# charlesq34/pointnet2

Hardware: AMD Instinct MI355X
Metric: point-clouds/sec for SA(FPS+ball+group) B=32 N=4096→1024 nsample=32 (higher is better)
Workload: dtype f32

## Files before the change

pointnet2_amd/csrc/fps_batch_body.h:

```cpp
#pragma once
#include "fps_pruned_body.h"

namespace pn2 {

constexpr int kBtCand = PN2_WAVE;
constexpr int kBtMaxW = 8;
#ifndef PN2_BT_UT
#define PN2_BT_UT 512
#endif
constexpr int kBtUT = PN2_BT_UT;
constexpr int kBtT = kBtUT + PN2_WAVE;
constexpr unsigned kBtEnd = 0x100u, kBtFill = 0x200u, kBtCountMask = 0xffu;

struct BtXchg {
    double list[kBtCand];
    unsigned cnt[kBtMaxW];
    unsigned bound[kBtMaxW];
    unsigned bmax;
    unsigned total;
    unsigned count;
    unsigned spare0;
    unsigned single;
    unsigned theta, vlast;
    unsigned spare1;
};
static_assert(sizeof(BtXchg) == 8 * kBtCand + 8 * kBtMaxW + 32, "the size the LDS budget of every geometry was measured with");
static_assert(sizeof(BtXchg) % 16 == 0 && offsetof(BtXchg, bmax) % 16 == 0, "16-byte rows");

__host__ __device__ constexpr size_t fps_batch_xchg_offset(int P, int UT = kBtUT) { return (fps_pruned_lds_bytes(P, UT) + 15) & ~(size_t)15; }
__host__ __device__ constexpr size_t fps_batch_lds_bytes(int P, int UT = kBtUT) { return fps_batch_xchg_offset(P, UT) + 2 * sizeof(BtXchg) + 16 * kBtCand; }

__device__ __forceinline__ float vmax_f32(float a, float b)
{
    float r;
    asm("v_max_f32 %0, %1, %2" : "=v"(r) : "v"(a), "v"(b));
    return r;
}
__device__ __forceinline__ float vmed3_f32(float a, float b, float c)
{
    float r;
    asm("v_med3_f32 %0, %1, %2, %3" : "=v"(r) : "v"(a), "v"(b), "v"(c));
    return r;
}

__device__ __forceinline__ int bt_wave_max_i32_lane63(int v)
{
#define PN2_BT_STEP(ctrl) v = max(v, __builtin_amdgcn_update_dpp(0, v, ctrl, 0xf, 0xf, true))
    PN2_BT_STEP(0xB1);
    PN2_BT_STEP(0x4E);
    PN2_BT_STEP(0x141);
    PN2_BT_STEP(0x140);
    PN2_BT_STEP(0x142);
    PN2_BT_STEP(0x143);
#undef PN2_BT_STEP
    return v;
}

__device__ __forceinline__ double kBtInvalidKey() { return -1.0; }

__device__ __forceinline__ void lds_max_u32(unsigned *p, unsigned v)
{
    asm volatile("ds_max_u32 %0, %1" :: "v"((unsigned)(size_t)p), "v"(v) : "memory");
}

__device__ __forceinline__ void lds_add_u32(unsigned *p, unsigned v)
{
    asm volatile("ds_add_u32 %0, %1" :: "v"((unsigned)(size_t)p), "v"(v) : "memory");
}

inline bool fps_batch_covers(int ranks) { return ranks > 512 && ranks <= 8192; }
#ifdef PN2_BT_LAB_NEVER_AUTO
inline bool fps_batch_pays(int, int) { return false; }
#else
inline bool fps_batch_pays(int ranks, int m) { return fps_batch_covers(ranks) && m >= 256; }
#endif

#ifdef PN2_BT_STATS
__device__ unsigned long long g_bt_stats[16];
#ifndef PN2_BT_STATS_FROM
#define PN2_BT_STATS_FROM 0
#endif
#define PN2_BT_STAT(i, v) do { if (lane == 0 && cloud == 0 && j >= PN2_BT_STATS_FROM) atomicAdd(&g_bt_stats[i], (unsigned long long)(v)); } while (0)
#define PN2_BT_CLOCK() __builtin_readcyclecounter()
#else
#define PN2_BT_STAT(i, v) do { } while (0)
#define PN2_BT_CLOCK() 0ll
#pragma clang diagnostic ignored "-Wunused-variable"
#endif

#ifndef PN2_BT_LIST_HI
#define PN2_BT_LIST_HI 36
#define PN2_BT_LIST_LO 20
#endif
#ifndef PN2_BT_EARLY
#define PN2_BT_EARLY 48
#endif
#ifndef PN2_BT_ASM_LOOP
#define PN2_BT_ASM_LOOP 1
#endif
#ifndef PN2_BT_RFL
#define PN2_BT_RFL 1
#endif
#ifndef PN2_BT_NOCTR
#define PN2_BT_NOCTR 1
#endif
#ifndef PN2_BT_FILL
#define PN2_BT_FILL 1
#endif
#ifndef PN2_BT_READ1
#define PN2_BT_READ1 1
#endif
#ifndef PN2_BT_CADD
#define PN2_BT_CADD 1
#endif
#ifndef PN2_BT_G0
#define PN2_BT_G0 0.10f
#endif
#ifndef PN2_BT_PACKED_FROM
#define PN2_BT_PACKED_FROM 16
#endif
#ifndef PN2_BT_SLOW_MIN
#define PN2_BT_SLOW_MIN 3
#define PN2_BT_QUICK 1
#define PN2_BT_SINGLE0 16
#define PN2_BT_SINGLE1 512
#endif

template <int P, int GS, bool PUBLISH, int UT = kBtUT>
__device__ __forceinline__ void fps_batch_body(int n, int m, int Q, int cloud, const float *__restrict__ xyz,
                                               int *__restrict__ out, float *__restrict__ out_xyz,
                                               unsigned long long *__restrict__ tagged, char *smem, unsigned tag = 1u)
{
    constexpr int W = UT / PN2_WAVE, NS = UT * P;
    constexpr int GW = P / GS;
    constexpr int CAP = kBtCand / W;
    constexpr int BT = UT + PN2_WAVE;
    static_assert((W * GW == 32 && (W == 4 || W == 8)) || (W == 8 && (GW == 2 || GW == 1)),
                  "32 groups on four or eight updater waves; 16 / 8 groups (2048 / 1024 rank slots) on eight");
    float4 *lds_rank = reinterpret_cast<float4 *>(smem + 256);
    BtXchg *xch = reinterpret_cast<BtXchg *>(smem + fps_batch_xchg_offset(P, UT));
    float4 *ring = reinterpret_cast<float4 *>(smem + fps_batch_xchg_offset(P, UT) + 2 * sizeof(BtXchg));

    const float *__restrict__ src = xyz + (size_t)cloud * n * 3;
    int *__restrict__ dst = out + (size_t)cloud * m;
    float *__restrict__ dxyz = out_xyz ? out_xyz + (size_t)cloud * m * 3 : nullptr;
    pn2_gu64 *gtag = PUBLISH ? (pn2_gu64 *)(tagged + (size_t)cloud * m) : nullptr;
    const int t = threadIdx.x;
    const int lane = t & 63;
    const int w = __builtin_amdgcn_readfirstlane(t >> 6);

    int j = 1;
    const int jE = min(PN2_BT_EARLY, m);
    int fill_k = -1;

    if (w == W) {
#ifndef PN2_NO_SETPRIO
        __builtin_amdgcn_s_setprio(3);
#endif
        for (int i = lane; i < (int)(2 * sizeof(BtXchg) / 4); i += PN2_WAVE) reinterpret_cast<unsigned *>(xch)[i] = 0u;
#if PN2_BT_READ1
        xch[0].list[lane] = kBtInvalidKey();
        xch[1].list[lane] = kBtInvalidKey();
#endif
        for (int i = 0; i < kPrPrologueBarriers; ++i) __syncthreads();
        long long e0 = 0;
        for (; j < jE; ++j) {
            if (j == 8) e0 = (long long)__builtin_readcyclecounter();
            __syncthreads();
        }
        const float round_cyc = jE >= 24 ? (float)((long long)__builtin_readcyclecounter() - e0) / (float)(jE - 8) : 1e30f;
        float bt_cyc = 0.f, bt_smp = 0.f;
        int bt_n = 0, bt_paid = 0, run = PN2_BT_SINGLE0, a_prev = 0, single_next = 0;
        long long qb = 0;
        float g = PN2_BT_G0;
        int par = 0;
        if (j < m)
        for (;;) {
            const long long q0 = PN2_BT_CLOCK();
#if PN2_BT_READ1
            xch[par ^ 1].list[lane] = kBtInvalidKey();
#endif
            {
                const long long qn = (long long)__builtin_readcyclecounter();
                if (bt_n > 0) {
                    bt_cyc = 0.75f * bt_cyc + (float)(qn - qb); bt_smp = 0.75f * bt_smp + (float)a_prev;
                    if (bt_n > PN2_BT_QUICK) {
                        if (bt_cyc > bt_smp * round_cyc * (bt_n > PN2_BT_SLOW_MIN ? 1.0f : 1.5f)) {
                            single_next = run;
                            run = min(2 * run, PN2_BT_SINGLE1);
                            bt_n = -1; bt_paid = 0; bt_cyc = 0.f; bt_smp = 0.f;
                        } else if (++bt_paid >= 8) {
                            run = PN2_BT_SINGLE0;
                        }
                    }
                }
                qb = qn;
                ++bt_n;
            }
            __syncthreads();
            const long long q1 = PN2_BT_CLOCK();
            BtXchg &X = xch[par];
            typedef float bt_f4 __attribute__((ext_vector_type(4)));
#if PN2_BT_READ1
            if (lane == 0) *reinterpret_cast<uint4 *>(&xch[par ^ 1].bmax) = make_uint4(0u, 0u, 0u, 0u);
            const uint2 bt2 = *reinterpret_cast<const uint2 *>(&X.bmax);
            const double key = X.list[lane];
            const unsigned lowc = (unsigned)__double2loint(key);
            const bt_f4 cand = *reinterpret_cast<const bt_f4 *>(&lds_rank[lowc]);
            const int boundb = __builtin_amdgcn_readfirstlane((int)bt2.x);
            const int total = __builtin_amdgcn_readfirstlane((int)bt2.y);
            int cval = __double2hiint(key);
#else
            if (lane == 0) __hip_atomic_store(&xch[par ^ 1].count, 0u, __ATOMIC_RELAXED, __HIP_MEMORY_SCOPE_WORKGROUP);
            const uint4 c4 = *reinterpret_cast<const uint4 *>(X.cnt), c5 = *reinterpret_cast<const uint4 *>(X.cnt + 4);
            const uint4 b4 = *reinterpret_cast<const uint4 *>(X.bound), b5 = *reinterpret_cast<const uint4 *>(X.bound + 4);
            const double key = X.list[lane];
            const unsigned cw = X.cnt[lane / CAP];
            const bool valid = (unsigned)(lane & (CAP - 1)) < cw;
            const unsigned lowc = valid ? (unsigned)__double2loint(key) : 0u;
            const bt_f4 cand = *reinterpret_cast<const bt_f4 *>(&lds_rank[lowc]);
            const int boundb = __builtin_amdgcn_readfirstlane((int)max(max(max(b4.x, b4.y), max(b4.z, b4.w)), max(max(b5.x, b5.y), max(b5.z, b5.w))));
            const int total = __builtin_amdgcn_readfirstlane((int)(c4.x + c4.y + c4.z + c4.w + c5.x + c5.y + c5.z + c5.w));
            int cval = valid ? __double2hiint(key) : (int)0xBF800000;
#endif
            const int clo = (int)lowc;
            int a = 0;
            int vlastb = 0;
            bool fill = false;
            const unsigned ring_base = (unsigned)(size_t)ring, count_addr = (unsigned)(size_t)&X.count;
            const long long q2 = PN2_BT_CLOCK();
            int bh;
            unsigned long long eq;
            auto argmax = [&]() __attribute__((always_inline)) {
                bh = __builtin_amdgcn_readlane(bt_wave_max_i32_lane63(cval), 63);
                eq = __ballot(cval == bh);
                if (__popcll(eq) != 1) {
                    PN2_BT_STAT(11, 1);
                    const double kq = cval == bh ? __hiloint2double(cval, clo) : -1.0;
                    const double km = wave_max_f64_lane63(kq);
                    const int ml = __builtin_amdgcn_readlane(__double2loint(km), 63);
                    eq = __ballot(cval == bh && clo == ml);
                    eq &= 0ull - eq;
                }
            };
            argmax();
            const int amax = min(m - j, kBtCand);
            unsigned raddr = ring_base, na = 1u;
            auto pick_counted = [&]() __attribute__((always_inline)) {
                for (;;) {
                    asm volatile("s_mov_b64 exec, %1\n\t"
                                 "ds_write_b128 %2, %3\n\t"
                                 "ds_write_b32 %4, %5\n\t"
                                 "v_mov_b32 %0, 0xbf800000\n\t"
                                 "s_mov_b64 exec, -1"
                                 : "+v"(cval) : "s"(eq), "v"(raddr), "v"(cand), "v"(count_addr), "v"(na) : "memory");
                    const int wl = (int)__builtin_ctzll(eq);
                    raddr += 16u; na += 1u;
                    a = __builtin_amdgcn_readfirstlane(a + 1);
                    vlastb = bh;
                    if (a >= amax) break;
                    const int ms = __builtin_amdgcn_readlane(bt_wave_max_i32_lane63(cval), 63);
                    const float sx = __int_as_float(__builtin_amdgcn_readlane(__float_as_int(cand.x), wl));
                    const float sy = __int_as_float(__builtin_amdgcn_readlane(__float_as_int(cand.y), wl));
                    const float sz = __int_as_float(__builtin_amdgcn_readlane(__float_as_int(cand.z), wl));
                    const float d = sqdist(cand.x, cand.y, cand.z, sx, sy, sz);
                    cval = __float_as_int(vmin_f32(d, __int_as_float(cval)));
                    if (ms < boundb) break;
                    eq = __ballot(cval == ms);
                    bh = ms;
                    if (__popcll(eq) != 1) {
                        PN2_BT_STAT(12, 1);
                        argmax();
                        if (bh < boundb) break;
                    }
                }
            };
#if PN2_BT_ASM_LOOP
#if PN2_BT_RFL
#define PN2_BT_A_WINNER_IN  "v_readfirstlane_b32 %[sx], %[cx]\n\tv_readfirstlane_b32 %[sy], %[cy]\n\tv_readfirstlane_b32 %[sz], %[cz]\n\t"
#define PN2_BT_A_LANE       ""
#define PN2_BT_A_SXY        ""
#define PN2_BT_A_SZ         ""
#else
#define PN2_BT_A_WINNER_IN  ""
#define PN2_BT_A_LANE       "s_ff1_i32_b64 %[wl], %[eq]\n\t"
#define PN2_BT_A_SXY        "v_readlane_b32 %[sx], %[cx], %[wl]\n\tv_readlane_b32 %[sy], %[cy], %[wl]\n\t"
#define PN2_BT_A_SZ         "v_readlane_b32 %[sz], %[cz], %[wl]\n\t"
#endif
#if PN2_BT_NOCTR
#define PN2_BT_A_COUNT      ""
#define PN2_BT_A_FULL       ""
#else
#define PN2_BT_A_COUNT      "s_add_i32 %[a], %[a], 1\n\t"
#define PN2_BT_A_FULL       "s_cmp_ge_i32 %[a], %[amax]\n\ts_cbranch_scc1 2f\n\t"
#endif
#if PN2_BT_CADD
#define PN2_BT_A_PUBCOUNT   "ds_add_u32 %[caddr], %[one]\n\t"
#define PN2_BT_A_NA         ""
#else
#define PN2_BT_A_PUBCOUNT   "ds_write_b32 %[caddr], %[na]\n\t"
#define PN2_BT_A_NA         "v_add_u32 %[na], 1, %[na]\n\t"
#endif
#if PN2_BT_CADD && PN2_BT_FILL
#define PN2_BT_A_HEAD       "0:\n\t"
#define PN2_BT_A_BH         "s_mov_b32 %[bh], %[ms]\n\t"
#define PN2_BT_A_MS         "+s"
#else
#define PN2_BT_A_HEAD       "s_branch 1f\n\t0:\n\ts_mov_b32 %[bh], %[ms]\n\t1:\n\t"
#define PN2_BT_A_BH         ""
#define PN2_BT_A_MS         "=&s"
#endif
#if PN2_BT_FILL
#define PN2_BT_A_ADDS_EARLY ""
#define PN2_BT_A_PAD_DPP    "v_add_u32 %[raddr], 16, %[raddr]\n\t" PN2_BT_A_NA PN2_BT_A_BH
#define PN2_BT_A_PAD        ""
#else
#define PN2_BT_A_ADDS_EARLY "v_add_u32 %[raddr], 16, %[raddr]\n\t" PN2_BT_A_NA
#define PN2_BT_A_PAD_DPP    "s_nop 1\n\t"
#define PN2_BT_A_PAD        "s_nop 0\n\t"
#endif
            const float cx = cand.x, cy = cand.y, cz = cand.z;
#if PN2_BT_NOCTR
            if (amax < kBtCand) pick_counted();
            else
#endif
            for (;;) {
                int reason, t_wl, t_sx, t_sy, t_sz, t_cnt;
                int t_ms = bh;
                int v_t;
                float v_dx, v_dy, v_dz;
                asm volatile(
                    PN2_BT_A_HEAD
                    "s_mov_b64 exec, %[eq]\n\t"
                    "ds_write_b128 %[raddr], %[cand]\n\t"
                    PN2_BT_A_PUBCOUNT
                    "v_mov_b32 %[cval], 0xbf800000\n\t"
                    PN2_BT_A_WINNER_IN
                    "s_mov_b64 exec, -1\n\t"
                    PN2_BT_A_LANE
                    PN2_BT_A_COUNT
                    PN2_BT_A_ADDS_EARLY
                    PN2_BT_A_FULL
                    PN2_BT_A_SXY
                    "v_max_i32_dpp %[t], %[cval], %[cval] quad_perm:[1,0,3,2] row_mask:0xf bank_mask:0xf bound_ctrl:0\n\t"
                    PN2_BT_A_SZ
                    "v_subrev_f32 %[dx], %[sx], %[cx]\n\t"
                    "v_subrev_f32 %[dy], %[sy], %[cy]\n\t"
                    "v_max_i32_dpp %[t], %[t], %[t] quad_perm:[2,3,0,1] row_mask:0xf bank_mask:0xf bound_ctrl:0\n\t"
                    "v_subrev_f32 %[dz], %[sz], %[cz]\n\t"
                    "v_mul_f32 %[dx], %[dx], %[dx]\n\t"
                    "v_max_i32_dpp %[t], %[t], %[t] row_half_mirror row_mask:0xf bank_mask:0xf bound_ctrl:0\n\t"
                    "v_mul_f32 %[dy], %[dy], %[dy]\n\t"
                    "v_mul_f32 %[dz], %[dz], %[dz]\n\t"
                    "v_max_i32_dpp %[t], %[t], %[t] row_mirror row_mask:0xf bank_mask:0xf bound_ctrl:0\n\t"
                    "v_add_f32 %[dx], %[dx], %[dy]\n\t"
                    "v_add_f32 %[dx], %[dx], %[dz]\n\t"
                    "v_max_i32_dpp %[t], %[t], %[t] row_bcast:15 row_mask:0xf bank_mask:0xf bound_ctrl:0\n\t"
                    PN2_BT_A_PAD_DPP
                    "v_max_i32_dpp %[t], %[t], %[t] row_bcast:31 row_mask:0xf bank_mask:0xf bound_ctrl:0\n\t"
                    "v_min_f32 %[cval], %[dx], %[cval]\n\t"
                    PN2_BT_A_PAD
                    "v_readlane_b32 %[ms], %[t], 63\n\t"
                    PN2_BT_A_PAD
                    "s_cmp_lt_i32 %[ms], %[bound]\n\t"
                    "s_cbranch_scc1 3f\n\t"
                    "v_cmp_eq_u32_e64 %[eq], %[ms], %[cval]\n\t"
                    "s_bcnt1_i32_b64 %[cnt], %[eq]\n\t"
                    "s_cmp_eq_u32 %[cnt], 1\n\t"
                    "s_cbranch_scc1 0b\n\t"
                    "s_mov_b32 %[reason], 2\n\t"
                    "s_branch 4f\n\t"
#if !PN2_BT_NOCTR
                    "2:\n\t"
                    "s_mov_b32 %[reason], 0\n\t"
                    "s_branch 4f\n\t"
#endif
                    "3:\n\t"
                    "s_mov_b32 %[reason], 1\n\t"
                    "4:"
                    : [cval] "+v"(cval), [raddr] "+v"(raddr), [na] "+v"(na), [eq] "+s"(eq), [bh] "+s"(bh),
#if !PN2_BT_NOCTR
                      [a] "+s"(a),
#endif
                      [reason] "=&s"(reason), [wl] "=&s"(t_wl), [sx] "=&s"(t_sx), [sy] "=&s"(t_sy), [sz] "=&s"(t_sz), [ms] PN2_BT_A_MS(t_ms), [cnt] "=&s"(t_cnt),
                      [t] "=&v"(v_t), [dx] "=&v"(v_dx), [dy] "=&v"(v_dy), [dz] "=&v"(v_dz)
                    : [cand] "v"(cand), [caddr] "v"(count_addr), [cx] "v"(cx), [cy] "v"(cy), [cz] "v"(cz), [amax] "s"(amax), [bound] "s"(boundb), [one] "v"(1u)
                    : "memory", "scc");
                vlastb = bh;
                if (reason != 2) break;
                PN2_BT_STAT(12, 1);
                argmax();
                if (bh < boundb) break;
            }
#if PN2_BT_NOCTR
#if PN2_BT_CADD
            a = (int)((unsigned)__builtin_amdgcn_readfirstlane((int)raddr) - ring_base) >> 4;
#else
            a = __builtin_amdgcn_readfirstlane((int)na) - 1;
#endif
#endif
#undef PN2_BT_A_WINNER_IN
#undef PN2_BT_A_LANE
#undef PN2_BT_A_SXY
#undef PN2_BT_A_SZ
#undef PN2_BT_A_COUNT
#undef PN2_BT_A_FULL
#undef PN2_BT_A_PUBCOUNT
#undef PN2_BT_A_NA
#undef PN2_BT_A_HEAD
#undef PN2_BT_A_BH
#undef PN2_BT_A_MS
#undef PN2_BT_A_ADDS_EARLY
#undef PN2_BT_A_PAD_DPP
#undef PN2_BT_A_PAD
#else
            pick_counted();
#endif
            if (vlastb == 0) { fill = true; fill_k = __builtin_amdgcn_readlane(__float_as_int(cand.w), (int)__builtin_ctzll(eq)); }
            const long long q3 = PN2_BT_CLOCK();
            if (total > PN2_BT_LIST_HI) g = fmaxf(g * 0.8f, 1.0f / 128.0f);
            else if (total < PN2_BT_LIST_LO) g = fminf(g * 1.25f, 0.5f);
            X.theta = __float_as_uint(__fmul_rn(__int_as_float(vlastb), 1.0f - g));
            X.vlast = (unsigned)vlastb;
            a_prev = a;
            int single = min(single_next, m - (j + a));
            if (single_next) { PN2_BT_STAT(13, single); PN2_BT_STAT(14, 1); }
            single_next = 0;
            single = __builtin_amdgcn_readfirstlane(single);
            X.single = (unsigned)single;
            if (lane == 0)
                __hip_atomic_store(&X.count, (unsigned)a | kBtEnd | (fill ? kBtFill : 0u), __ATOMIC_RELEASE, __HIP_MEMORY_SCOPE_WORKGROUP);
            PN2_BT_STAT(0, 1); PN2_BT_STAT(1, a); PN2_BT_STAT(4, total); PN2_BT_STAT(6, q2 - q1); PN2_BT_STAT(7, q3 - q2); PN2_BT_STAT(8, q1 - q0);
            j = __builtin_amdgcn_readfirstlane(j + a);
            if (fill || j >= m) break;
            for (int i = 0; i < single; ++i) __syncthreads();
            j += single;
            if (j >= m) break;
            par ^= 1;
        }
    } else {
        PrSlots<P> S;
        fps_pruned_prologue<P, GS, UT>(n, Q, src, smem, S);
        pn2_f2 (&xx)[P / 2] = S.xx;
        pn2_f2 (&yy)[P / 2] = S.yy;
        pn2_f2 (&zz)[P / 2] = S.zz;
        float (&md)[P] = S.md;
        unsigned (&low)[P] = S.low;
        float blx, bly, blz, bhx, bhy, bhz;
        {
            const float *gbox = reinterpret_cast<const float *>(smem + 256 + (size_t)16 * NS + (size_t)kPrHistRows * kPrBins * 4);
            const float *o = gbox + (w * GW + (lane & (GW - 1))) * 8;
            blx = o[0]; bly = o[1]; blz = o[2]; bhx = o[4]; bhy = o[5]; bhz = o[6];
        }
        pn2_f2 sxy = {0.f, 0.f}, syy = {0.f, 0.f}, szk = {0.f, 0.f};
        auto update_group = [&](auto gic) __attribute__((always_inline)) {
            constexpr int gi = decltype(gic)::value;
            constexpr int H = GS / 2;
            pn2_f2 dx[H], dy[H], dz[H];
#pragma unroll
            for (int h = 0; h < H; ++h) dx[h] = pk_sub_bcast_lo(xx[gi * H + h], sxy);
#pragma unroll
            for (int h = 0; h < H; ++h) dy[h] = pk_sub_bcast_lo(yy[gi * H + h], syy);
#pragma unroll
            for (int h = 0; h < H; ++h) dz[h] = pk_sub_bcast_lo(zz[gi * H + h], szk);
#pragma unroll
            for (int h = 0; h < H; ++h) dx[h] = pk_mul(dx[h], dx[h]);
#pragma unroll
            for (int h = 0; h < H; ++h) dy[h] = pk_mul(dy[h], dy[h]);
#pragma unroll
            for (int h = 0; h < H; ++h) dz[h] = pk_mul(dz[h], dz[h]);
#pragma unroll
            for (int h = 0; h < H; ++h) dx[h] = pk_add(dx[h], dy[h]);
#pragma unroll
            for (int h = 0; h < H; ++h) dx[h] = pk_add(dx[h], dz[h]);
#pragma unroll
            for (int h = 0; h < H; ++h) {
                const int p0 = gi * GS + 2 * h;
                md[p0] = vmin_f32(dx[h].x, md[p0]);
                md[p0 + 1] = vmin_f32(dx[h].y, md[p0 + 1]);
            }
        };
        auto update_all = [&]() __attribute__((always_inline)) {
            update_group(std::integral_constant<int, 0>());
            if constexpr (GW >= 2) update_group(std::integral_constant<int, 1>());
            if constexpr (GW >= 4) { update_group(std::integral_constant<int, 2>()); update_group(std::integral_constant<int, 3>()); }
            if constexpr (GW == 8) {
                update_group(std::integral_constant<int, 4>()); update_group(std::integral_constant<int, 5>());
                update_group(std::integral_constant<int, 6>()); update_group(std::integral_constant<int, 7>());
            }
        };
        {
            const float4 s = lds_rank[NS - 1];
            sxy.x = s.x; syy.x = s.y; szk.x = s.z;
            update_all();
        }
        if (t == 0) {
            dst[0] = 0;
            if (PUBLISH) __hip_atomic_store(gtag, (unsigned long long)tag << 32, __ATOMIC_RELAXED, __HIP_MEMORY_SCOPE_AGENT);
        }
        unsigned vlastb = __float_as_uint(1e38f);
        unsigned thetab = __float_as_uint(1e38f);
        auto single_rounds = [&](const int jend) __attribute__((always_inline)) {
            double *partial = reinterpret_cast<double *>(smem);
            for (; j < jend; ++j) {
                double kd[P];
#pragma unroll
                for (int p = 0; p < P; ++p) kd[p] = __hiloint2double(__float_as_int(md[p]), (int)low[p]);
#pragma unroll
                for (int st = 1; st < P; st <<= 1)
#pragma unroll
                    for (int i = 0; i + st < P; i += 2 * st)
                        asm("v_max_f64 %0, %1, %2" : "=v"(kd[i]) : "v"(kd[i]), "v"(kd[i + st]));
                const double wd = wave_max_f64_lane63(kd[0]);
                double *slot = partial + (j & 1) * W;
                if (lane == 63) slot[w] = wd;
                __syncthreads();
                double key[W];
#pragma unroll
                for (int i = 0; i < W; ++i) key[i] = slot[i];
#pragma unroll
                for (int st = 1; st < W; st <<= 1)
#pragma unroll
                    for (int i = 0; i + st < W; i += 2 * st)
                        asm("v_max_f64 %0, %1, %2" : "=v"(key[i]) : "v"(key[i]), "v"(key[i + st]));
                vlastb = (unsigned)__double2hiint(key[0]);
                const float4 s = lds_rank[(unsigned)__double2loint(key[0])];
                if (t == 0) {
                    const int k = __float_as_int(s.w);
                    dst[j] = k;
                    if (PUBLISH)
                        __hip_atomic_store(gtag + j, ((unsigned long long)tag << 32) | (unsigned long long)(unsigned)k, __ATOMIC_RELAXED,
                                           __HIP_MEMORY_SCOPE_AGENT);
                }
                if constexpr (P >= PN2_BT_PACKED_FROM) {
                    sxy.x = s.x; syy.x = s.y; szk.x = s.z;
                    update_all();
                } else {
#pragma unroll
                    for (int p = 0; p < P; ++p) {
                        const float d = p & 1 ? sqdist(xx[p / 2].y, yy[p / 2].y, zz[p / 2].y, s.x, s.y, s.z)
                                              : sqdist(xx[p / 2].x, yy[p / 2].x, zz[p / 2].x, s.x, s.y, s.z);
                        md[p] = vmin_f32(d, md[p]);
                    }
                }
            }
            thetab = __float_as_uint(__fmul_rn(__uint_as_float(vlastb), 1.0f - PN2_BT_G0));
        };
        if (jE > 1) single_rounds(jE);
        int par = 0;
        if (j < m)
        for (;;) {
            BtXchg &X = xch[par];
            const long long u0 = PN2_BT_CLOCK();
            double kl;
            float sec;
            {
                double kd[P];
                float hv[P / 2], lv[P / 2];
#pragma unroll
                for (int p = 0; p < P; ++p) kd[p] = __hiloint2double(__float_as_int(md[p]), (int)low[p]);
#pragma unroll
                for (int i = 0; i < P / 2; ++i) { hv[i] = vmax_f32(md[2 * i], md[2 * i + 1]); lv[i] = vmin_f32(md[2 * i], md[2 * i + 1]); }
#pragma unroll
                for (int st = 1; st < P; st <<= 1)
#pragma unroll
                    for (int i = 0; i + st < P; i += 2 * st)
                        asm("v_max_f64 %0, %1, %2" : "=v"(kd[i]) : "v"(kd[i]), "v"(kd[i + st]));
#pragma unroll
                for (int st = 1; st < P / 2; st <<= 1)
#pragma unroll
                    for (int i = 0; i + st < P / 2; i += 2 * st) {
                        const float ll = vmax_f32(lv[i], lv[i + st]);
                        lv[i] = vmed3_f32(hv[i], hv[i + st], ll);
                        hv[i] = vmax_f32(hv[i], hv[i + st]);
                    }
                kl = kd[0];
                sec = lv[0];
            }
            const unsigned vb = (unsigned)__double2hiint(kl);
            unsigned long long mask = __ballot(vb >= thetab);
            int cnt = __popcll(mask);
            unsigned thb = thetab;
            bool exact = false;
            if (cnt > CAP) {
                unsigned lob = thetab, hib = vlastb + 1u;
                for (int it = 0; it < 16; ++it) {
                    const unsigned mid = lob + ((hib - lob) >> 1);
                    if (mid == lob) break;
                    const unsigned long long mk = __ballot(vb >= mid);
                    const int c = __popcll(mk);
                    PN2_BT_STAT(3, 1);
                    if (c > CAP) lob = mid;
                    else if (c == 0) hib = mid;
                    else { mask = mk; cnt = c; thb = mid; break; }
                }
                exact = cnt > CAP;
            } else if (cnt == 0) {
                exact = true;
            }
            if (exact) {
                PN2_BT_STAT(2, 1);
                const double wk = wave_max_f64_lane63(kl);
                const int bh = __builtin_amdgcn_readlane(__double2hiint(wk), 63), bl = __builtin_amdgcn_readlane(__double2loint(wk), 63);
                unsigned long long mk = __ballot(__double2hiint(kl) == bh && __double2loint(kl) == bl);
                mk &= 0ull - mk;
                if (cnt != 0) thb = (unsigned)bh + 1u;
                mask = mk;
                cnt = 1;
            }
            if ((mask >> lane) & 1ull) {
                const int pos = __builtin_amdgcn_mbcnt_hi((unsigned)(mask >> 32), __builtin_amdgcn_mbcnt_lo((unsigned)mask, 0u));
                X.list[w * CAP + pos] = kl;
#if PN2_BT_READ1
                lds_max_u32(&X.bmax, __float_as_uint(sec) + 1u);
#else
                lds_max_u32(&X.bound[w], __float_as_uint(sec) + 1u);
#endif
            }
            if (lane == 0) {
#if PN2_BT_READ1
                lds_add_u32(&X.total, (unsigned)cnt);
                lds_max_u32(&X.bmax, thb);
#else
                X.cnt[w] = (unsigned)cnt;
                lds_max_u32(&X.bound[w], thb);
#endif
            }
            const long long u1 = PN2_BT_CLOCK();
            asm volatile("s_waitcnt lgkmcnt(0)" ::: "memory");
            __syncthreads();
            const long long u2 = PN2_BT_CLOCK();
#if !PN2_BT_READ1
            if (lane == 0) xch[par ^ 1].bound[w] = 0u;
#endif
            int done = 0;
            unsigned c;
            const float thr = __fadd_rn(__fmul_rn(__uint_as_float(vlastb), 1.00001f), 1e-30f);
            for (;;) {
                c = __hip_atomic_load(&X.count, __ATOMIC_ACQUIRE, __HIP_MEMORY_SCOPE_WORKGROUP);
                c = (unsigned)__builtin_amdgcn_readfirstlane((int)c);
                const int avail = (int)(c & kBtCountMask);
                if (avail == done) {
                    if (c & kBtEnd) break;
                    __builtin_amdgcn_s_sleep(1);
                    continue;
                }
                constexpr int CH = PN2_WAVE / GW;
                constexpr unsigned long long kStride = GW == 8 ? 0x0101010101010101ull : GW == 4 ? 0x1111111111111111ull
                                                       : GW == 2 ? 0x5555555555555555ull : ~0ull;
                const int np = min(avail - done, CH);
                const int pi = lane / GW;
                const float4 s = ring[done + (pi < np ? pi : 0)];
                const float ax = __fsub_rn(s.x, __builtin_amdgcn_fmed3f(s.x, blx, bhx));
                const float ay = __fsub_rn(s.y, __builtin_amdgcn_fmed3f(s.y, bly, bhy));
                const float az = __fsub_rn(s.z, __builtin_amdgcn_fmed3f(s.z, blz, bhz));
                const float bd = __fadd_rn(__fadd_rn(__fmul_rn(ax, ax), __fmul_rn(ay, ay)), __fmul_rn(az, az));
                unsigned long long touched = ~__ballot(bd >= thr);
                if (np * GW < 64) touched &= (1ull << (np * GW)) - 1ull;
                if (touched) {
                    if (2 * __popcll(touched) >= GW * np) {
                        for (int p = 0; p < np; ++p) {
                            sxy.x = __int_as_float(__builtin_amdgcn_readlane(__float_as_int(s.x), p * GW));
                            syy.x = __int_as_float(__builtin_amdgcn_readlane(__float_as_int(s.y), p * GW));
                            szk.x = __int_as_float(__builtin_amdgcn_readlane(__float_as_int(s.z), p * GW));
                            update_all();
                        }
                    } else {
                        auto one_group = [&](auto gic) __attribute__((always_inline)) {
                            constexpr int g8 = decltype(gic)::value;
                            unsigned long long mg = touched & (kStride << g8);
                            while (mg) {
                                const int sl = (int)__builtin_ctzll(mg) & ~(GW - 1);
                                mg &= mg - 1ull;
                                sxy.x = __int_as_float(__builtin_amdgcn_readlane(__float_as_int(s.x), sl));
                                syy.x = __int_as_float(__builtin_amdgcn_readlane(__float_as_int(s.y), sl));
                                szk.x = __int_as_float(__builtin_amdgcn_readlane(__float_as_int(s.z), sl));
                                PN2_BT_STAT(5, 1);
                                update_group(gic);
                            }
                        };
                        one_group(std::integral_constant<int, 0>());
                        if constexpr (GW >= 2) one_group(std::integral_constant<int, 1>());
                        if constexpr (GW >= 4) { one_group(std::integral_constant<int, 2>()); one_group(std::integral_constant<int, 3>()); }
                        if constexpr (GW == 8) {
                            one_group(std::integral_constant<int, 4>()); one_group(std::integral_constant<int, 5>());
                            one_group(std::integral_constant<int, 6>()); one_group(std::integral_constant<int, 7>());
                        }
                    }
                }
                done += np;
            }
            const long long u3 = PN2_BT_CLOCK();
            if (w == 0) { PN2_BT_STAT(9, u1 - u0); PN2_BT_STAT(10, u3 - u2); }
            const int a = (int)(c & kBtCountMask);
            if (w == 0 && lane < a) {
                const int k = __float_as_int(ring[lane].w);
                dst[j + lane] = k;
                if (PUBLISH)
                    __hip_atomic_store(gtag + (j + lane), ((unsigned long long)tag << 32) | (unsigned long long)(unsigned)k, __ATOMIC_RELAXED,
                                       __HIP_MEMORY_SCOPE_AGENT);
            }
            if (c & kBtFill) fill_k = __float_as_int(ring[a - 1].w);
            j += a;
            if ((c & kBtFill) || j >= m) break;
            thetab = X.theta;
            vlastb = X.vlast;
            const int single = __builtin_amdgcn_readfirstlane((int)X.single);
            if (single) {
                single_rounds(min(j + single, m));
                if (j >= m) break;
            }
            par ^= 1;
        }
    }
    if (fill_k >= 0) {
        for (int i = j + t; i < m; i += BT) {
            dst[i] = fill_k;
            if (PUBLISH)
                __hip_atomic_store(gtag + i, ((unsigned long long)tag << 32) | (unsigned long long)(unsigned)fill_k, __ATOMIC_RELAXED,
                                   __HIP_MEMORY_SCOPE_AGENT);
        }
    }
    fps_gather_epilogue<BT>(m, src, dst, dxyz);
}

}
```

Measured before the change: 149,700.

## Use max3/med3 second-best selection, exec-masked list writes, group-major lane layout

Computes the per-thread second-best distance with v_max3/v_med3 triplet reductions and a pairwise f64 max tree instead of the pairwise hi/lo ladder. When the candidate count fits the per-wave capacity, it writes the list entry and updates the bound counters through a single inline-asm block with an explicit exec mask. Lanes are also remapped so each group owns a contiguous lane range, which lets touched-point iteration use 32-bit masks per group. Together these cut ALU and scalar overhead in the FPS batch loop, at the cost of raw exec manipulation in inline asm that the compiler cannot reason about.

```diff
diff --git a/pointnet2_amd/csrc/fps_batch_body.h b/pointnet2_amd/csrc/fps_batch_body.h
--- a/pointnet2_amd/csrc/fps_batch_body.h
+++ b/pointnet2_amd/csrc/fps_batch_body.h
@@ -43,6 +43,43 @@
     return r;
 }
 
+__device__ __forceinline__ float vmax3_f32(float a, float b, float c)
+{
+    float r;
+    asm("v_max3_f32 %0, %1, %2, %3" : "=v"(r) : "v"(a), "v"(b), "v"(c));
+    return r;
+}
+
+template <int P>
+__device__ __forceinline__ float bt_second_best(const float (&v)[P])
+{
+    static_assert(P == 2 || P == 4 || P == 8 || P == 16, "slots per updater thread");
+    constexpr int NT = P / 3, REM = P % 3, K = NT + (REM == 2 ? 1 : 0), KF = K >= 3 ? 3 : K;
+    float h[K > 0 ? K : 1], l[K > 0 ? K : 1];
+#pragma unroll
+    for (int i = 0; i < NT; ++i) { h[i] = vmax3_f32(v[3 * i], v[3 * i + 1], v[3 * i + 2]); l[i] = vmed3_f32(v[3 * i], v[3 * i + 1], v[3 * i + 2]); }
+    if constexpr (REM == 2) { h[NT] = vmax_f32(v[P - 2], v[P - 1]); l[NT] = vmin_f32(v[P - 2], v[P - 1]); }
+    int k = K;
+#pragma unroll
+    while (k > 3) {
+        const float hm = vmed3_f32(h[k - 3], h[k - 2], h[k - 1]), lm = vmax3_f32(l[k - 3], l[k - 2], l[k - 1]);
+        h[k - 3] = vmax3_f32(h[k - 3], h[k - 2], h[k - 1]);
+        l[k - 3] = vmax_f32(hm, lm);
+        k -= 2;
+    }
+    if constexpr (REM == 1) {
+        if constexpr (KF == 3) {
+            const float hm = vmed3_f32(h[0], h[1], h[2]), lm = vmax3_f32(l[0], l[1], l[2]);
+            h[0] = vmax3_f32(h[0], h[1], h[2]);
+            l[0] = vmax_f32(hm, lm);
+        }
+        return vmed3_f32(h[0], l[0], v[P - 1]);
+    } else {
+        if constexpr (KF == 3) return vmax_f32(vmed3_f32(h[0], h[1], h[2]), vmax3_f32(l[0], l[1], l[2]));
+        else return l[0];
+    }
+}
+
 __device__ __forceinline__ int bt_wave_max_i32_lane63(int v)
 {
 #define PN2_BT_STEP(ctrl) v = max(v, __builtin_amdgcn_update_dpp(0, v, ctrl, 0xf, 0xf, true))
@@ -76,7 +113,7 @@
 #endif
 
 #ifdef PN2_BT_STATS
-__device__ unsigned long long g_bt_stats[16];
+__device__ unsigned long long g_bt_stats[24];
 #ifndef PN2_BT_STATS_FROM
 #define PN2_BT_STATS_FROM 0
 #endif
@@ -112,6 +149,15 @@
 #endif
 #ifndef PN2_BT_CADD
 #define PN2_BT_CADD 1
+#endif
+#ifndef PN2_BT_SEC3
+#define PN2_BT_SEC3 1
+#endif
+#ifndef PN2_BT_CTAIL
+#define PN2_BT_CTAIL 1
+#endif
+#ifndef PN2_BT_GBITS
+#define PN2_BT_GBITS 1
 #endif
 #ifndef PN2_BT_G0
 #define PN2_BT_G0 0.10f
@@ -135,6 +181,8 @@
     constexpr int GW = P / GS;
     constexpr int CAP = kBtCand / W;
     constexpr int BT = UT + PN2_WAVE;
+    constexpr int CH = PN2_WAVE / GW;
+    constexpr bool GB = PN2_BT_GBITS && GW > 1;
     static_assert((W * GW == 32 && (W == 4 || W == 8)) || (W == 8 && (GW == 2 || GW == 1)),
                   "32 groups on four or eight updater waves; 16 / 8 groups (2048 / 1024 rank slots) on eight");
     float4 *lds_rank = reinterpret_cast<float4 *>(smem + 256);
@@ -449,7 +497,7 @@
         float blx, bly, blz, bhx, bhy, bhz;
         {
             const float *gbox = reinterpret_cast<const float *>(smem + 256 + (size_t)16 * NS + (size_t)kPrHistRows * kPrBins * 4);
-            const float *o = gbox + (w * GW + (lane & (GW - 1))) * 8;
+            const float *o = gbox + (w * GW + (GB ? lane / CH : (lane & (GW - 1)))) * 8;
             blx = o[0]; bly = o[1]; blz = o[2]; bhx = o[4]; bhy = o[5]; bhz = o[6];
         }
         pn2_f2 sxy = {0.f, 0.f}, syy = {0.f, 0.f}, szk = {0.f, 0.f};
@@ -548,6 +596,7 @@
         };
         if (jE > 1) single_rounds(jE);
         int par = 0;
+        long long uend = 0;
         if (j < m)
         for (;;) {
             BtXchg &X = xch[par];
@@ -556,9 +605,18 @@
             float sec;
             {
                 double kd[P];
+#pragma unroll
+                for (int p = 0; p < P; ++p) kd[p] = __hiloint2double(__float_as_int(md[p]), (int)low[p]);
+#if PN2_BT_SEC3
+#pragma unroll
+                for (int st = 1; st < P; st <<= 1)
+#pragma unroll
+                    for (int i = 0; i + st < P; i += 2 * st)
+                        asm("v_max_f64 %0, %1, %2" : "=v"(kd[i]) : "v"(kd[i]), "v"(kd[i + st]));
+                kl = kd[0];
+                sec = bt_second_best<P>(md);
+#else
                 float hv[P / 2], lv[P / 2];
-#pragma unroll
-                for (int p = 0; p < P; ++p) kd[p] = __hiloint2double(__float_as_int(md[p]), (int)low[p]);
 #pragma unroll
                 for (int i = 0; i < P / 2; ++i) { hv[i] = vmax_f32(md[2 * i], md[2 * i + 1]); lv[i] = vmin_f32(md[2 * i], md[2 * i + 1]); }
 #pragma unroll
@@ -576,11 +634,31 @@
                     }
                 kl = kd[0];
                 sec = lv[0];
+#endif
             }
             const unsigned vb = (unsigned)__double2hiint(kl);
             unsigned long long mask = __ballot(vb >= thetab);
             int cnt = __popcll(mask);
             unsigned thb = thetab;
+#if PN2_BT_CTAIL && PN2_BT_READ1
+            static_assert(offsetof(BtXchg, total) == offsetof(BtXchg, bmax) + 4, "one address register for both words");
+            auto list_write = [&](const unsigned long long mk, const int c, const unsigned th) __attribute__((always_inline)) {
+                const unsigned pos = __builtin_amdgcn_mbcnt_hi((unsigned)(mk >> 32), __builtin_amdgcn_mbcnt_lo((unsigned)mk, 0u));
+                asm volatile("s_mov_b64 exec, %[mk]\n\t"
+                             "ds_write_b64 %[la], %[kl]\n\t"
+                             "ds_max_u32 %[ba], %[sec1]\n\t"
+                             "s_mov_b64 exec, 1\n\t"
+                             "ds_add_u32 %[ba], %[c] offset:4\n\t"
+                             "ds_max_u32 %[ba], %[th]\n\t"
+                             "s_mov_b64 exec, -1"
+                             :: [mk] "s"(mk), [la] "v"((unsigned)(size_t)&X.list[w * CAP] + 8u * pos), [kl] "v"(kl),
+                                [ba] "v"((unsigned)(size_t)&X.bmax), [sec1] "v"(__float_as_uint(sec) + 1u), [c] "v"((unsigned)c), [th] "v"(th)
+                             : "memory");
+            };
+            if ((unsigned)(cnt - 1) < (unsigned)CAP) {
+                list_write(mask, cnt, thb);
+            } else {
+#endif
             bool exact = false;
             if (cnt > CAP) {
                 unsigned lob = thetab, hib = vlastb + 1u;
@@ -608,6 +686,11 @@
                 mask = mk;
                 cnt = 1;
             }
+#if PN2_BT_CTAIL && PN2_BT_READ1
+                list_write(((unsigned long long)(unsigned)__builtin_amdgcn_readfirstlane((int)(mask >> 32)) << 32) |
+                               (unsigned)__builtin_amdgcn_readfirstlane((int)mask), cnt, thb);
+            }
+#else
             if ((mask >> lane) & 1ull) {
                 const int pos = __builtin_amdgcn_mbcnt_hi((unsigned)(mask >> 32), __builtin_amdgcn_mbcnt_lo((unsigned)mask, 0u));
                 X.list[w * CAP + pos] = kl;
@@ -626,7 +709,9 @@
                 lds_max_u32(&X.bound[w], thb);
 #endif
             }
+#endif
             const long long u1 = PN2_BT_CLOCK();
+            if (w == 0 && uend) PN2_BT_STAT(15, u1 - uend);
             asm volatile("s_waitcnt lgkmcnt(0)" ::: "memory");
             __syncthreads();
             const long long u2 = PN2_BT_CLOCK();
@@ -642,41 +727,63 @@
                 const int avail = (int)(c & kBtCountMask);
                 if (avail == done) {
                     if (c & kBtEnd) break;
+                    if (w == 0) PN2_BT_STAT(17, 1);
                     __builtin_amdgcn_s_sleep(1);
                     continue;
                 }
-                constexpr int CH = PN2_WAVE / GW;
+                if (w == 0) PN2_BT_STAT(16, 1);
                 constexpr unsigned long long kStride = GW == 8 ? 0x0101010101010101ull : GW == 4 ? 0x1111111111111111ull
                                                        : GW == 2 ? 0x5555555555555555ull : ~0ull;
                 const int np = min(avail - done, CH);
-                const int pi = lane / GW;
+                const int pi = GB ? (lane & (CH - 1)) : lane / GW;
                 const float4 s = ring[done + (pi < np ? pi : 0)];
                 const float ax = __fsub_rn(s.x, __builtin_amdgcn_fmed3f(s.x, blx, bhx));
                 const float ay = __fsub_rn(s.y, __builtin_amdgcn_fmed3f(s.y, bly, bhy));
                 const float az = __fsub_rn(s.z, __builtin_amdgcn_fmed3f(s.z, blz, bhz));
                 const float bd = __fadd_rn(__fadd_rn(__fmul_rn(ax, ax), __fmul_rn(ay, ay)), __fmul_rn(az, az));
                 unsigned long long touched = ~__ballot(bd >= thr);
-                if (np * GW < 64) touched &= (1ull << (np * GW)) - 1ull;
+                if constexpr (GB) {
+                    constexpr unsigned kRep = CH == 32 ? 1u : CH == 16 ? 0x00010001u : 0x01010101u;
+                    if (np < CH) { const unsigned vm = ((1u << np) - 1u) * kRep; touched &= ((unsigned long long)vm << 32) | vm; }
+                } else {
+                    if (np * GW < 64) touched &= (1ull << (np * GW)) - 1ull;
+                }
                 if (touched) {
                     if (2 * __popcll(touched) >= GW * np) {
+                        if (w == 0) PN2_BT_STAT(18, GW * np);
                         for (int p = 0; p < np; ++p) {
-                            sxy.x = __int_as_float(__builtin_amdgcn_readlane(__float_as_int(s.x), p * GW));
-                            syy.x = __int_as_float(__builtin_amdgcn_readlane(__float_as_int(s.y), p * GW));
-                            szk.x = __int_as_float(__builtin_amdgcn_readlane(__float_as_int(s.z), p * GW));
+                            const int sl = GB ? p : p * GW;
+                            sxy.x = __int_as_float(__builtin_amdgcn_readlane(__float_as_int(s.x), sl));
+                            syy.x = __int_as_float(__builtin_amdgcn_readlane(__float_as_int(s.y), sl));
+                            szk.x = __int_as_float(__builtin_amdgcn_readlane(__float_as_int(s.z), sl));
                             update_all();
                         }
                     } else {
                         auto one_group = [&](auto gic) __attribute__((always_inline)) {
                             constexpr int g8 = decltype(gic)::value;
-                            unsigned long long mg = touched & (kStride << g8);
-                            while (mg) {
-                                const int sl = (int)__builtin_ctzll(mg) & ~(GW - 1);
-                                mg &= mg - 1ull;
-                                sxy.x = __int_as_float(__builtin_amdgcn_readlane(__float_as_int(s.x), sl));
-                                syy.x = __int_as_float(__builtin_amdgcn_readlane(__float_as_int(s.y), sl));
-                                szk.x = __int_as_float(__builtin_amdgcn_readlane(__float_as_int(s.z), sl));
-                                PN2_BT_STAT(5, 1);
-                                update_group(gic);
+                            if constexpr (GB) {
+                                unsigned mg = (unsigned)(touched >> (g8 * CH));
+                                if constexpr (CH < 32) mg &= (1u << CH) - 1u;
+                                while (mg) {
+                                    const int sl = (int)__builtin_ctz(mg);
+                                    asm("s_bitset0_b32 %0, %1" : "+s"(mg) : "s"(sl));
+                                    sxy.x = __int_as_float(__builtin_amdgcn_readlane(__float_as_int(s.x), sl));
+                                    syy.x = __int_as_float(__builtin_amdgcn_readlane(__float_as_int(s.y), sl));
+                                    szk.x = __int_as_float(__builtin_amdgcn_readlane(__float_as_int(s.z), sl));
+                                    PN2_BT_STAT(5, 1);
+                                    update_group(gic);
+                                }
+                            } else {
+                                unsigned long long mg = touched & (kStride << g8);
+                                while (mg) {
+                                    const int sl = (int)__builtin_ctzll(mg) & ~(GW - 1);
+                                    mg &= mg - 1ull;
+                                    sxy.x = __int_as_float(__builtin_amdgcn_readlane(__float_as_int(s.x), sl));
+                                    syy.x = __int_as_float(__builtin_amdgcn_readlane(__float_as_int(s.y), sl));
+                                    szk.x = __int_as_float(__builtin_amdgcn_readlane(__float_as_int(s.z), sl));
+                                    PN2_BT_STAT(5, 1);
+                                    update_group(gic);
+                                }
                             }
                         };
                         one_group(std::integral_constant<int, 0>());
@@ -691,6 +798,7 @@
                 done += np;
             }
             const long long u3 = PN2_BT_CLOCK();
+            uend = u3;
             if (w == 0) { PN2_BT_STAT(9, u1 - u0); PN2_BT_STAT(10, u3 - u2); }
             const int a = (int)(c & kBtCountMask);
             if (w == 0 && lane < a) {
```

After: 153,800 (median of 6 runs). 2.8% higher.
